# Infinidat/slimfastq

Measured on AMD Instinct MI355X. Metric: MB/s FASTQ compressed, higher is better.
Workload: dtype u8/u32 integer; 1 GPU; synthetic 10M x 150 bp Illumina reads per GPU, full qlts+gens+recs, frozen tables (one chain per lane), -l 3; level=3, block_reads=1024, prior_step=-1, blocks_per_gpu=9766, tables=frozen, chains_per_gpu=253906, raw_bytes_per_gpu=3702038404, parallelism=1 GPU

## Files before the change

slimfastq_amd/csrc/chains.hip:

```cpp
#include "kernels.h"
#include "dev_chain.h"
#include "dev_walk.h"
typedef u32 __attribute__((aligned(1))) u32_any;

#define LAST_QLT 63u
#define QROW_BYTES 256u
#define B2_INIT 0x03030303u

#define QDEC_ROW 72u
__device__ __forceinline__ void qdec_store(u16* row, u32 s, u32 cum) {
    if (s) row[8 + s - 1] = (u16)cum;
    if ((s & 7u) == 0) row[s >> 3] = (u16)cum;
    if (s == 63) row[8 + 63] = 0;
}
__global__ __launch_bounds__(256) void k_qlt_frozen_rows(const u32* __restrict__ rows66, u32 q_rows, u32* __restrict__ qrows, u16* __restrict__ qdec) {
    const u32 lane = threadIdx.x & 63;
    const u32 ctx = blockIdx.x * 4 + (threadIdx.x >> 6);
    if (ctx >= q_rows) return;
    const u32* r = rows66 + (size_t)ctx * 66;
    const u32 slot = r[lane], iend = r[65];
    if (iend == 0) {
        qrows[(size_t)ctx * 64 + lane] = (lane << 10) | (1024u << 16);
        if (qdec) qdec_store(qdec + (size_t)ctx * QDEC_ROW, lane, lane << 10);
        return;
    }
    const u32 sym = slot >> 16, fslot = lane < iend ? (slot & 0xffffu) : 0u;
    const u32 f = (u32)__builtin_amdgcn_ds_permute((int)((lane < iend ? sym : lane) * 4), (int)fslot);
    const u32 x = f + 1;
    u32 S = x;
#pragma unroll
    for (int d = 32; d > 0; d >>= 1) S += (u32)__shfl_xor((int)S, d, 64);
    u32 g = (x << 16) / S;
    g = g ? g : 1u;
    u32 sum = g, best = (g << 6) | (63u - lane);
#pragma unroll
    for (int d = 32; d > 0; d >>= 1) {
        sum += (u32)__shfl_xor((int)sum, d, 64);
        const u32 o = (u32)__shfl_xor((int)best, d, 64); best = o > best ? o : best;
    }
    if (lane == 63u - (best & 63u)) g += 65536u - sum;
    u32 incl = g;
#pragma unroll
    for (int d = 1; d < 64; d <<= 1) { const u32 o = (u32)__shfl_up((int)incl, d, 64); if (lane >= (u32)d) incl += o; }
    qrows[(size_t)ctx * 64 + lane] = (incl - g) | (g << 16);
    if (qdec) qdec_store(qdec + (size_t)ctx * QDEC_ROW, lane, incl - g);
}
void launch_qlt_frozen_rows(const u32* rows66, u32 q_rows, u32* qrows, u16* qdec, hipStream_t st) {
    hipLaunchKernelGGL(k_qlt_frozen_rows, dim3((q_rows + 3) / 4), dim3(256), 0, st, rows66, q_rows, qrows, qdec);
}

#define QH_SYMS 48u
#define QH_ROW_U16 50u
#define QH_MAP_BYTES(q_rows) ((q_rows) / 32u * 8u)
#define QH_EMPTY 0xFFFFFFFFu
__global__ __launch_bounds__(256) void k_hot_totals(const u32* __restrict__ hist, const u32* __restrict__ rows66, u32 q_rows, u32* __restrict__ ctot) {
    const u32 lane = threadIdx.x & 63;
    const u32 ctx = blockIdx.x * 4 + (threadIdx.x >> 6);
    if (ctx >= q_rows) return;
    u32 c = hist[(size_t)ctx * 64 + lane];
#pragma unroll
    for (int d = 32; d > 0; d >>= 1) c += (u32)__shfl_xor((int)c, d, 64);
    const u32 iend = rows66[(size_t)ctx * 66 + 65];
    if (lane == 0) ctot[ctx] = (iend != 0 && iend <= QH_SYMS) ? c : 0u;
}
__global__ __launch_bounds__(1024) void k_hot_select(const u32* __restrict__ ctot, u32 q_rows, u32 want, uint2* __restrict__ map, u32* __restrict__ info) {
    __shared__ u32 red[16];
    __shared__ u32 wbits[2048];
    const u32 t = threadIdx.x, lane = t & 63, wave = t >> 6;
    const u32 nwords = q_rows / 32u;
    u32 c[64];
    u32 mx = 0;
#pragma unroll
    for (u32 k = 0; k < 64; k++) {
        const u32 ctx = k * 1024u + t;
        c[k] = ctx < q_rows ? ctot[ctx] : 0u;
        mx = c[k] > mx ? c[k] : mx;
    }
    auto block_sum = [&](u32 v) {
#pragma unroll
        for (int d = 32; d > 0; d >>= 1) v += (u32)__shfl_xor((int)v, d, 64);
        __syncthreads();
        if (lane == 0) red[wave] = v;
        __syncthreads();
        u32 s2 = 0;
        for (u32 w = 0; w < 16; w++) s2 += red[w];
        return s2;
    };
    auto block_max = [&](u32 v) {
#pragma unroll
        for (int d = 32; d > 0; d >>= 1) { const u32 o = (u32)__shfl_xor((int)v, d, 64); v = o > v ? o : v; }
        __syncthreads();
        if (lane == 0) red[wave] = v;
        __syncthreads();
        u32 s2 = 0;
        for (u32 w = 0; w < 16; w++) s2 = red[w] > s2 ? red[w] : s2;
        return s2;
    };
    u32 lo = 1, hi = block_max(mx) + 1u;
    while (lo < hi) {
        const u32 mid = lo + (hi - lo) / 2u;
        u32 n = 0;
#pragma unroll
        for (u32 k = 0; k < 64; k++) n += c[k] >= mid;
        if (block_sum(n) <= want) hi = mid; else lo = mid + 1u;
    }
    const u32 T = lo;
#pragma unroll
    for (u32 k = 0; k < 64; k++) {
        const u64 m = __ballot(c[k] >= T);
        if (lane == 0) { wbits[k * 32u + wave * 2u] = (u32)m; wbits[k * 32u + wave * 2u + 1u] = (u32)(m >> 32); }
    }
    __syncthreads();
    const u32 b0 = 2u * t < nwords ? wbits[2u * t] : 0u, b1 = 2u * t + 1u < nwords ? wbits[2u * t + 1u] : 0u;
    const u32 mine = (u32)__popc(b0) + (u32)__popc(b1);
    u32 inc = mine;
#pragma unroll
    for (int d = 1; d < 64; d <<= 1) { const u32 o = (u32)__shfl_up((int)inc, d, 64); if (lane >= (u32)d) inc += o; }
    __syncthreads();
    if (lane == 63) red[wave] = inc;
    __syncthreads();
    u32 before = 0, all = 0;
    for (u32 w = 0; w < 16; w++) { const u32 v = red[w]; before += w < wave ? v : 0u; all += v; }
    const u32 rank = before + inc - mine;
    if (t == 0) info[0] = all;
    if (2u * t < nwords) map[2u * t] = make_uint2(b0, rank);
    if (2u * t + 1u < nwords) map[2u * t + 1u] = make_uint2(b1, rank + (u32)__popc(b0));
}
__global__ __launch_bounds__(256) void k_hot_image(const uint2* __restrict__ map, const u32* __restrict__ qrows, u32 q_rows, u16* __restrict__ rows) {
    const u32 lane = threadIdx.x & 63;
    const u32 ctx = blockIdx.x * 4 + (threadIdx.x >> 6);
    if (ctx >= q_rows) return;
    const uint2 mr = map[ctx >> 5];
    const u32 bit = 1u << (ctx & 31u);
    if (!(mr.x & bit)) return;
    const u32 slot = mr.y + (u32)__popc(mr.x & (bit - 1u));
    if (lane < QH_ROW_U16) rows[(size_t)slot * QH_ROW_U16 + lane] = lane <= QH_SYMS ? (u16)FZ_CUM(qrows[(size_t)ctx * 64 + lane]) : (u16)0;
}
void launch_hot_rows(const u32* hist, const u32* rows66, const u32* qrows, u32 q_rows, u32 want, u32* ctot, u8* img, u32* info, hipStream_t st) {
    hipLaunchKernelGGL(k_hot_totals, dim3((q_rows + 3) / 4), dim3(256), 0, st, hist, rows66, q_rows, ctot);
    hipLaunchKernelGGL(k_hot_select, dim3(1), dim3(1024), 0, st, (const u32*)ctot, q_rows, want, reinterpret_cast<uint2*>(img), info);
    hipLaunchKernelGGL(k_hot_image, dim3((q_rows + 3) / 4), dim3(256), 0, st, reinterpret_cast<const uint2*>(img), qrows, q_rows,
                       reinterpret_cast<u16*>(img + QH_MAP_BYTES(q_rows)));
}

#define QHD_ROW_U16 8u
#define QHD_MAX_ROWS 6000u
__global__ __launch_bounds__(256) void k_hot_totals_prior(const u32* __restrict__ rows66, u32 q_rows, u32* __restrict__ ctot) {
    const u32 ctx = blockIdx.x * 256 + threadIdx.x;
    if (ctx >= q_rows) return;
    const u32 iend = rows66[(size_t)ctx * 66 + 65];
    ctot[ctx] = iend != 0 ? rows66[(size_t)ctx * 66 + 64] + 1u : 0u;
}
__global__ __launch_bounds__(256) void k_hot_image_dec(const uint2* __restrict__ map, const u16* __restrict__ qdec, u32 q_rows, u16* __restrict__ rows) {
    const u32 ctx = blockIdx.x * 256 + threadIdx.x;
    if (ctx >= q_rows) return;
// ... 584 lines not shown
            if (w0 | w1) slice[i] = c;
            if (rows_out && last_chunk) rows_out[((size_t)b << sb) + i] = gen_row_of(c, step);
        }
        if (last_chunk) break;
        __syncthreads();
    }
    if (tid == 0) fill[b] = 0;
}
GenBins gen_bins_plan(u32 g_bits, u64 max_keys) {
    GenBins gb; gb.bins = nullptr; gb.fill = nullptr;
    gb.g_bits = g_bits;
    gb.batch = max_keys < GEN_BIN_BATCH ? (max_keys ? max_keys : 1) : GEN_BIN_BATCH;
    const u32 nb = 1u << (g_bits - gb_slice_bits(g_bits));
    gb.cap = (u32)((2ull * ((gb.batch + nb - 1) / nb) + 4096ull + 63ull) & ~63ull);
    gb.bins_bytes = (u64)gb.cap * 2ull * nb; gb.fill_bytes = 4ull * nb;
    return gb;
}
void launch_gen_count_binned(const ChainArgs& a, u32 b0, u32 b1, u64 nrec_range, u32 max_line, const GenBins& gb, u32* cnt, u32* rows_out, u32 step,
                             hipStream_t st, u32 sub) {
    const u32 g_bits = gb.g_bits, sb = gb_slice_bits(g_bits), nb = 1u << (g_bits - sb), cap = gb.cap;
    const u32 dyn2 = (2u << sb) * 4u;
    static u32 allowed = 0;
    if (dyn2 > 65536u && dyn2 > allowed) { (void)hipFuncSetAttribute(reinterpret_cast<const void*>(&k_gen_bin_count), hipFuncAttributeMaxDynamicSharedMemorySize, (int)dyn2); allowed = dyn2; }
    if (nrec_range) {
        u32 stride = gen_count_stride(nrec_range);
        if (sub == 1) { stride *= GEN_PRE; sub = 0; }
        u32 seg_len = 0;
        if (max_line >= 64u) {
            const u64 nsel = (nrec_range + stride - 1) / stride;
            for (u32 sl = 32u; sl < max_line && sl <= 512u; sl *= 2u)
                if (nsel * ((max_line + sl - 1) / sl) <= 524288ull) { seg_len = sl; break; }
        }
        if (!seg_len && max_line > 1024u) seg_len = 512u;
        const u32 segs = seg_len ? (max_line + seg_len - 1) / seg_len : 1u;
        const u64 lanes = ((nrec_range + stride - 1) / stride) * segs;
        const u64 per_lane = seg_len ? seg_len : (max_line ? max_line : 1u);
        u64 lanes_per_batch = gb.batch / per_lane; if (!lanes_per_batch) lanes_per_batch = 1;
        lanes_per_batch = (lanes_per_batch + GB_T - 1) / GB_T * GB_T;
        const u32 dyn1 = (GB_TILE + 2u * nb) * 4u;
        for (u64 id0 = 0; id0 < lanes; id0 += lanes_per_batch) {
            const u64 id1 = id0 + lanes_per_batch < lanes ? id0 + lanes_per_batch : lanes;
            const bool last = id1 >= lanes;
            hipLaunchKernelGGL(k_gen_bin, dim3((u32)((id1 - id0 + GB_T - 1) / GB_T)), dim3(GB_T), dyn1, st, a, b0, b1, stride, seg_len, segs, sub, id0, id1, g_bits, gb.bins, gb.fill, cap, cnt);
            hipLaunchKernelGGL(k_gen_bin_count, dim3(nb), dim3(1024), dyn2, st, (const u16*)gb.bins, gb.fill, cap, g_bits, cnt, last ? rows_out : nullptr, step);
        }
    } else if (rows_out) hipLaunchKernelGGL(k_gen_bin_count, dim3(nb), dim3(1024), dyn2, st, (const u16*)gb.bins, gb.fill, cap, g_bits, cnt, rows_out, step);
}

__global__ __launch_bounds__(256) void k_gen_rows(const u32* __restrict__ cnt, u32* __restrict__ rows, u64 nctx, u32 step) {
    const u64 c = (u64)blockIdx.x * 256 + threadIdx.x;
    if (c >= nctx) return;
    const uint4 n = *reinterpret_cast<const uint4*>(cnt + c * 4);
    u64 f0 = 3 + (u64)step * n.x, f1 = 3 + (u64)step * n.y, f2 = 3 + (u64)step * n.z, f3 = 3 + (u64)step * n.w;
    while ((f0 | f1 | f2 | f3) > 255) {
        f0 = (f0 >> 1) | (f0 & 1); f1 = (f1 >> 1) | (f1 & 1); f2 = (f2 >> 1) | (f2 & 1); f3 = (f3 >> 1) | (f3 & 1);
    }
    rows[c] = (u32)f0 | (u32)f1 << 8 | (u32)f2 << 16 | (u32)f3 << 24;
}
void launch_gen_rows(const u32* cnt, u32* rows, u64 nctx, u32 step, hipStream_t st) {
    hipLaunchKernelGGL(k_gen_rows, dim3((u32)((nctx + 255) / 256)), dim3(256), 0, st, cnt, rows, nctx, step);
}

__device__ __forceinline__ const u32* gen_rows_of(const ChainArgs& a, u32 b) {
    if (!a.g_ngen) return nullptr;
    u32 g = 0;
    while (g + 1 < a.g_ngen && b >= a.g_bound[g + 1]) g++;
    return a.g_rows[g];
}

#define GEN_RING 8
template <int THREADS, bool FLAT>
__global__ __launch_bounds__(THREADS) void k_gen_encode_c(ChainArgs a, u32 c0, u32 c1 ) {
    __shared__ u32 rcp[FLAT ? 1 : 1024];
    __shared__ u8 lut[256];
    __shared__ u32 ring[LaneEncB<THREADS, GEN_RING>::LDS_DWORDS];
    if constexpr (!FLAT) for (u32 i = threadIdx.x; i < 1024; i += THREADS) rcp[i] = i ? fz_recip(i) : 0u;
    for (u32 i = threadIdx.x; i < 256; i += THREADS) lut[i] = (u8)(gen_code_of(i) | (is_lower_base(i) ? 0x20u : 0u));
    __syncthreads();
    const u32 c = c0 + blockIdx.x * THREADS + threadIdx.x;
    const bool live = c < c1;
    ChainPos cp; cp.b = 0; cp.r0 = 0; cp.nrec = 0; cp.sub_lo = cp.sub_len = 0; cp.seg = 0; cp.nseg = 1;
    if (live) { cp = chain_pos(a, c); chain_seg_encode(a, cp); }
    const BlockDesc* d = &a.m.blocks[cp.b];
    LaneEncB<THREADS, GEN_RING> rc; u32 cap = 0;
    u8* outp = live ? chain_region(a, cp, SFQ_S_GEN, 3, 4, cap) : nullptr;
    rc.init(ring, threadIdx.x, outp, cap);
    const u32* rows = (!FLAT && live) ? gen_rows_of(a, cp.b) : nullptr;
    u32 illegal = 0;
    if (a.flat_quads && (FLAT || !__any(rows != nullptr))) {
        illegal = walk_bases_q(a, cp.r0, cp.nrec, live ? d->solid : 0u, lut,
            [&](u32 sym, u32 k) { const u32 bits = 2u * k; rc.encode_bits_if(k ? ~0u : 0u, sym & ((1u << bits) - 1u), 1u, bits); rc.drain(); },
            a.exc_flag, cp.sub_lo, cp.sub_len);
    } else if (FLAT || !__any(rows != nullptr)) {
        const u32 r12 = fz_recip(12u);
        illegal = walk_bases_b(a, cp.r0, cp.nrec, live ? d->solid : 0u, 0u, lut, [&](u32, u32) {},
            [&](u32, u32 code, u32 vm) { rc.encode_if(vm, 3u * code, 3u, 12u, r12); },
            [&]() { rc.drain(); }, a.exc_flag, cp.sub_lo, cp.sub_len);
    } else if constexpr (!FLAT) {
        const u32* rp = rows ? rows : a.g_init;
        const u32 mask = (live && rows) ? (1u << d->gen_bits) - 1u : 0u;
        u32 rv[16];
        illegal = walk_bases_b(a, cp.r0, cp.nrec, live ? d->solid : 0u, mask, lut,
            [&](u32 j, u32 ctx) { rv[j] = rp[ctx]; },
            [&](u32 j, u32 code, u32 vm) {
                const u32 v = rv[j];
                const u32 f0 = v & 0xff, f1 = (v >> 8) & 0xff, f2 = (v >> 16) & 0xff, f3 = v >> 24;
                const u32 tot = (f0 + f1) + (f2 + f3);
                const u32 below = v & ((1u << (8 * code)) - 1u);
                const u32 cum = (below & 0xff) + ((below >> 8) & 0xff) + (below >> 16);
                rc.encode_if(vm, cum, (v >> (8 * code)) & 0xff, tot, rcp[tot]);
            },
            [&]() { rc.drain(); }, a.exc_flag, cp.sub_lo, cp.sub_len);
    }
    if (live) {
        a.csz[c] = rc.finish();
        if (rc.err & 2) atomicMax(&a.m.blocks[cp.b].status, (u32)(-SFQ_E_OVERFLOW));
        else if (rc.err) atomicMax(&a.m.blocks[cp.b].status, (u32)(-SFQ_E_CORRUPT));
        if (illegal) atomicMax(&a.m.blocks[cp.b].status, (u32)(-SFQ_E_GENCHAR));
    }
}
__device__ __forceinline__ uint4 gp_below(u32 n) {
    const u64 lo = n >= 8u ? ~0ull : (1ull << (8u * n)) - 1ull;
    const u64 hi = n >= 16u ? ~0ull : n <= 8u ? 0ull : (1ull << (8u * (n - 8u))) - 1ull;
    return make_uint4((u32)lo, (u32)(lo >> 32), (u32)hi, (u32)(hi >> 32));
}
__device__ __forceinline__ uint4 gp_load16(const u8* buf, u64 nbytes, long long at) {
    if (at >= 0 && (u64)at + 16u <= nbytes) return load16(buf, nbytes, (u64)at);
    u32 w[4] = {0, 0, 0, 0};
    for (u32 i = 0; i < 16; i++) { const long long p = at + (long long)i; if (p >= 0 && (u64)p < nbytes) w[i >> 2] |= (u32)buf[p] << ((i & 3) * 8); }
    return make_uint4(w[0], w[1], w[2], w[3]);
}
__device__ __forceinline__ u32 gp_codes(u32 w, u32 valid, u32& odd, u32& ill) {
    const u32 s1 = w >> 1;
    u32 cd = (s1 ^ (w >> 2)) & 0x03030303u;
    const u32 want = __builtin_amdgcn_perm(0u, 0x47544341u, s1 & 0x03030303u);
    odd = 0; ill = 0;
    if ((want ^ w) & valid) {
        cd = 0;
#pragma unroll
        for (u32 i = 0; i < 4; i++) {
            const u32 ch = (w >> (8u * i)) & 0xffu, g = gen_code_of(ch);
            cd |= (g & 3u) << (8u * i);
            if ((valid >> (8u * i)) & 0xffu) {
                if (g > 3u || is_lower_base(ch)) odd |= 0x80u << (8u * i);
                if (g & 0x10u) ill = 1;
            }
        }
    }
    return cd & valid & 0x03030303u;
}
__device__ __forceinline__ u32 gp_fold(u32 cd) { return cd | (cd >> 6); }
__device__ __forceinline__ u32 gp_nib(u32 t) { return ((t >> 7) * 0x01020408u) >> 24; }
__device__ __forceinline__ u32 gp_bits16(u32 o0, u32 o1, u32 o2, u32 o3) { return gp_nib(o0) | gp_nib(o1) << 4 | gp_nib(o2) << 8 | gp_nib(o3) << 12; }
__global__ __launch_bounds__(256) void k_gen_pack_raw(ChainArgs a, u32 c0, u32 c1) {
    const u32 lane = threadIdx.x & 63u;
    const u32 c = c0 + blockIdx.x * 4u + (threadIdx.x >> 6);
    if (c >= c1) return;
    ChainPos cp = chain_pos(a, c); chain_seg_encode(a, cp);
    const u32 solid = a.m.blocks[cp.b].solid;
    u32 cap = 0;
    u32* out = reinterpret_cast<u32*>(chain_region(a, cp, SFQ_S_GEN, 3, 4, cap));
    const u8* buf = a.st_off ? a.st_buf : a.m.fq;
    const u64 nbytes = a.st_off ? a.st_bytes : a.nbytes;
    u32 done = 0;
    u32 carry = 0;
    u32 illegal = 0;
    for (u32 k0 = 0; k0 < cp.nrec; k0 += 64u) {
        const u32 k = k0 + lane;
        u64 b0 = 0, b1 = 0;
        if (k < cp.nrec) {
            const u64 r = cp.r0 + k;
            if (a.st_off) { b0 = a.st_off[r]; b1 = b0 + a.st_len[r]; }
            else { b0 = a.m.line_off[4 * r + 1] + solid; b1 = a.m.line_off[4 * r + 2] - 1; }
            if (cp.sub_len) {
                if (b1 < b0) b1 = b0;
                const u64 lo = b0 + cp.sub_lo;
                b0 = lo < b1 ? lo : b1;
                b1 = b0 + cp.sub_len < b1 ? b0 + cp.sub_len : b1;
            }
            if (b1 < b0) b1 = b0;
        }
        const u32 len = (u32)(b1 - b0);
        u32 inc = len;
#pragma unroll
        for (int d = 1; d < 64; d <<= 1) { const u32 o = (u32)__shfl_up((int)inc, d, 64); if (lane >= (u32)d) inc += o; }
        const u32 st = inc - len;
        const u32 tot = (u32)__shfl((int)inc, 63, 64);
        const u32 end = done + tot;
        const bool last_chunk = k0 + 64u >= cp.nrec;
        const u32 t0 = done >> 4, t1 = (end + 15u) >> 4;
        for (u32 tb = t0; tb < t1; tb += 64u) {
            const u32 t = tb + lane;
            const u32 d0 = 16u * t;
            const u32 lo = d0 > done ? d0 : done, hi = d0 + 16u < end ? d0 + 16u : end;
            u32 kr = 0;
#pragma unroll
            for (u32 s = 32; s > 0; s >>= 1) { const u32 sk = (u32)__shfl((int)st, (int)(kr + s), 64); if (sk + done <= lo) kr += s; }
            uint4 w = make_uint4(0, 0, 0, 0);
            u32 pos = lo;
            while (__any(pos < hi)) {
                const u32 ks = kr & 63u;
                const u32 sk = (u32)__shfl((int)st, (int)ks, 64) + done, lk = (u32)__shfl((int)len, (int)ks, 64);
                const u64 bk = (u64)__shfl((unsigned long long)b0, (int)ks, 64);
                const u32 e = sk + lk < hi ? sk + lk : hi;
                if (pos < hi && e > pos) {
                    const u32 j = pos - d0;
                    const uint4 v = gp_load16(buf, nbytes, (long long)(bk + (pos - sk)) - (long long)j);
                    const uint4 m0 = gp_below(j), m1 = gp_below(j + (e - pos));
                    w.x = (w.x & ~(m1.x & ~m0.x)) | (v.x & m1.x & ~m0.x);
                    w.y = (w.y & ~(m1.y & ~m0.y)) | (v.y & m1.y & ~m0.y);
                    w.z = (w.z & ~(m1.z & ~m0.z)) | (v.z & m1.z & ~m0.z);
                    w.w = (w.w & ~(m1.w & ~m0.w)) | (v.w & m1.w & ~m0.w);
                    pos = e;
                }
                kr++;
            }
            const bool any = lo < hi;
            const uint4 va = gp_below(any ? hi - d0 : 0u), vb = gp_below(any ? lo - d0 : 0u);
            const uint4 vm = make_uint4(va.x & ~vb.x, va.y & ~vb.y, va.z & ~vb.z, va.w & ~vb.w);
            u32 o0, o1, o2, o3, i0, i1, i2, i3;
            const u32 f0 = gp_fold(gp_codes(w.x, vm.x, o0, i0)), f1 = gp_fold(gp_codes(w.y, vm.y, o1, i1));
            const u32 f2 = gp_fold(gp_codes(w.z, vm.z, o2, i2)), f3 = gp_fold(gp_codes(w.w, vm.w, o3, i3));
            illegal |= i0 | i1 | i2 | i3;
            u32 p01 = __builtin_amdgcn_perm(f1, f0, 0x06020400u), p23 = __builtin_amdgcn_perm(f3, f2, 0x06020400u);
            p01 |= p01 >> 12; p23 |= p23 >> 12;
            u32 code = __builtin_amdgcn_perm(p23, p01, 0x05040100u);
            if (t == t0) code |= carry;
            u32 odd = gp_bits16(o0, o1, o2, o3);
            if (a.exc_flag) {
                while (__any(odd != 0u)) {
                    const u32 jb = odd ? (u32)__builtin_ctz(odd) : 0u;
                    u32 ko = 0;
#pragma unroll
                    for (u32 s = 32; s > 0; s >>= 1) { const u32 sk = (u32)__shfl((int)st, (int)(ko + s), 64); if (sk + done <= d0 + jb) ko += s; }
                    const u32 ke = (u32)__shfl((int)inc, (int)ko, 64) + done;
                    if (odd) {
                        a.exc_flag[cp.r0 + k0 + ko] = 1;
                        odd &= ke - d0 >= 16u ? 0u : ~((1u << (ke - d0)) - 1u);
                    }
                }
            }
            const bool held = t == t1 - 1u && (end & 15u) && !last_chunk;
            if (t < t1 && !held && 4u * t < cap) out[t] = code;
            if (!last_chunk) carry = (end & 15u) ? (u32)__shfl((int)code, (int)((t1 - 1u - tb) & 63u), 64) : 0u;
        }
        done = end;
    }
    if (lane == 0) {
        const u32 n = (done + 3u) >> 2;
        a.csz[c] = n;
        if (n > cap) atomicMax(&a.m.blocks[cp.b].status, (u32)(-SFQ_E_OVERFLOW));
    }
    if (__any(illegal != 0u) && lane == 0) atomicMax(&a.m.blocks[cp.b].status, (u32)(-SFQ_E_GENCHAR));
}
void launch_gen_encode_c(const ChainArgs& a, hipStream_t st, u32 c0, u32 c1, bool flat) {
    constexpr int T = 256;
    if (!c1 || c1 > a.geo.nchains) c1 = a.geo.nchains;
    if (c1 <= c0) return;
    if (a.flat_raw) { hipLaunchKernelGGL(k_gen_pack_raw, dim3((c1 - c0 + 3) / 4), dim3(256), 0, st, a, c0, c1); return; }
    const dim3 grid((c1 - c0 + T - 1) / T);
    if (flat) hipLaunchKernelGGL((k_gen_encode_c<T, true>), grid, dim3(T), 0, st, a, c0, c1);
    else hipLaunchKernelGGL((k_gen_encode_c<T, false>), grid, dim3(T), 0, st, a, c0, c1);
}

__device__ __forceinline__ u32 b2_pick(u32 v, LaneDecQ& rc, const u32* rcp) {
    const u32 f0 = v & 0xff, f1 = (v >> 8) & 0xff, f2 = (v >> 16) & 0xff, f3 = v >> 24;
    const u32 c1 = f0, c2 = f0 + f1, c3 = c2 + f2, tot = c3 + f3;
    u32 r;
    const u32 prob = rc.get_freq(tot, rcp[tot], r);
    const u32 b = (prob >= c1 ? 1u : 0u) + (prob >= c2 ? 1u : 0u) + (prob >= c3 ? 1u : 0u);
    const u32 cum = b == 0 ? 0u : b == 1 ? c1 : b == 2 ? c2 : c3;
    rc.decode(r, cum, (v >> (8 * b)) & 0xff);
    return b;
}
template <int THREADS>
__global__ __launch_bounds__(THREADS) void k_gen_decode_c(ChainArgs a, DecodeArgs da, u32 c0, u32 c1 ) {
    __shared__ u32 rcp[1024];
    for (u32 i = threadIdx.x; i < 1024; i += THREADS) rcp[i] = i ? fz_recip(i) : 0u;
    __syncthreads();
    const u32 c = c0 + blockIdx.x * THREADS + threadIdx.x;
    if (c >= c1) return;
    ChainPos cp = chain_pos(a, c);
    const BlockDesc* d = &a.m.blocks[cp.b];
    LaneDecQ rc; rc.init(da.streams + a.coff[c], a.csz[c], reinterpret_cast<const u8*>(a.qesc));
    const u32* rows = gen_rows_of(a, cp.b);
    const u32 alphabet = d->solid ? 0x33323130u  : 0x54474341u ;
    const u32 mask = (1u << d->gen_bits) - 1u;
    const u32 INIT = 0x007616c7u;
    const u32 r12 = fz_recip(12u);
    u32 n_next = cp.nrec ? da.slen[cp.r0] : 0u; u64 off_next = cp.nrec ? da.soff[cp.r0] : 0ull;
    if (a.seg_len) {
        const u32 ql = da.qlen[cp.r0];
        seg_range(cp, ql > n_next ? ql : n_next);
        const u64 lo = cp.sub_lo < n_next ? cp.sub_lo : n_next;
        n_next = (u32)(n_next - lo < cp.sub_len ? n_next - lo : cp.sub_len); off_next += lo;
    }
    const u8* const raw = da.streams + a.coff[c]; const u32 raw_n = a.csz[c];
    u32 racc = 0, rnb = 0, rat = 0, rbad = 0;
    for (u32 k = 0; k < cp.nrec; k++) {
        const u32 llen = n_next; const u64 off = off_next;
        if (k + 1 < cp.nrec) { n_next = da.slen[cp.r0 + k + 1]; off_next = da.soff[cp.r0 + k + 1]; }
        LaneOut32 out; out.begin(da.seq_stage + off);
        u32 last = INIT;
        if (a.flat_raw) {
            for (u32 i = 0; i < llen; i++) {
                if (rnb == 0) {
                    if (rat + 4u <= raw_n) { racc = *reinterpret_cast<const u32_any*>(raw + rat); rat += 4u; rnb = 32u; }
                    else if (rat < raw_n) { racc = raw[rat++]; rnb = 8u; }
                    else { rbad = 1; racc = 0; rnb = 32u; }
                }
                out.put((alphabet >> (8u * (racc & 3u))) & 0xffu);
                racc >>= 2; rnb -= 2u;
            }
        } else
        if (rows) {
            u32 v = rows[last & mask];
            for (u32 i = 0; i < llen; i++) {
                const uint4 cand = *reinterpret_cast<const uint4*>(rows + ((last << 2) & mask));
                rc.top_up();
                const u32 b = b2_pick(v, rc, rcp);
                out.put((alphabet >> (8 * b)) & 0xff);
                last = (last << 2) | b;
                v = b == 0 ? cand.x : b == 1 ? cand.y : b == 2 ? cand.z : cand.w;
            }
        } else if (a.flat_quads) {
            for (u32 i = 0; i < llen; i += 4u) {
                const u32 k = llen - i < 4u ? llen - i : 4u;
                rc.top_up();
                u32 r;
                const u32 S = rc.get_freq_bits(2u * k, r);
                rc.decode1(r, S, 1u);
                for (u32 j = 0; j < k; j++) out.put((alphabet >> (8u * ((S >> (2u * j)) & 3u))) & 0xffu);
            }
        } else {
            for (u32 i = 0; i < llen; i++) {
                rc.top_up();
                u32 r;
                const u32 prob = rc.get_freq(12u, r12, r);
                const u32 b = (prob >= 3u ? 1u : 0u) + (prob >= 6u ? 1u : 0u) + (prob >= 9u ? 1u : 0u);
                rc.decode1(r, 3u * b, 3u);
                out.put((alphabet >> (8 * b)) & 0xff);
            }
        }
        out.end();
    }
    if (a.flat_raw) { if (rbad || rat != raw_n || (rnb >= 8u) || racc) atomicMax(&a.m.blocks[cp.b].status, (u32)(-SFQ_E_CORRUPT)); }
    else
    if (rc.err) atomicMax(&a.m.blocks[cp.b].status, (u32)(-SFQ_E_CORRUPT));
}
void launch_gen_decode_c(const ChainArgs& a, const DecodeArgs& da, u32 c0, u32 c1, hipStream_t st) {
    constexpr int T = 256;
    if (c1 > a.geo.nchains) c1 = a.geo.nchains;
    if (c1 <= c0) return;
    hipLaunchKernelGGL(k_gen_decode_c<T>, dim3((c1 - c0 + T - 1) / T), dim3(T), 0, st, a, da, c0, c1);
}

#include "dev_rec_lane.h"
#include "dev_wave.h"

struct RecChainPos { u32 b; u64 r0; u32 nrec; };
__device__ __forceinline__ RecChainPos rec_chain_pos(const ChainArgs& a, u32 c) {
    RecChainPos p;
    p.b = c / a.rgeo.cpb;
    const u32 j = c - p.b * a.rgeo.cpb;
    const BlockDesc* d = &a.m.blocks[p.b];
    const u32 k0 = j * a.rgeo.chain_reads;
    p.nrec = k0 < d->nrec ? (d->nrec - k0 < a.rgeo.chain_reads ? d->nrec - k0 : a.rgeo.chain_reads) : 0u;
    p.r0 = d->rec0 + k0;
    return p;
}
__device__ __forceinline__ u8* rec_chain_region(const ChainArgs& a, const RecChainPos& p, u32& cap) {
    const BlockDesc* d = &a.m.blocks[p.b];
    const u64 t0 = a.m.line_off[4 * d->rec0], tc = a.m.line_off[4 * p.r0], te = a.m.line_off[4 * (p.r0 + p.nrec)];
    const u64 lo = ((tc - t0) * 3 / 2 + 3) & ~3ull, hi = ((te - t0) * 3 / 2) & ~3ull;
    cap = hi > lo ? (u32)(hi - lo) : 0u;
    return a.m.arena + d->out_off[SFQ_S_REC] + lo;
}

#define REC_HBUF 128u
#define REC_LDS_ROWS 8u
struct RecFrozenEnc {
    static constexpr bool inband = true;
    const u32* rows; LaneEnc rc;
    u8* lbuf;
    const u16* lmap; const u32* lrows;
    __device__ __forceinline__ void record(u32) {}
    __device__ __forceinline__ const u8* stage(const u8* g, u32 n, u32 k) {
        if (n + 1 > REC_HBUF) return g;
        u8* dst = lbuf + (k & 1u) * REC_HBUF;
        const u32 nw = (n + 4) / 4;
#pragma unroll 8
        for (u32 i = 0; i < nw; i++) reinterpret_cast<u32*>(dst)[i] = reinterpret_cast<const u32_any*>(g)[i];
        return dst;
    }
    __device__ __forceinline__ void put(u32 row, u32 sym) {
        const u32 slot = lmap[row];
        const u32 e = slot != 0xFFFFu ? lrows[slot * 256 + sym] : rows[(size_t)row * 256 + sym];
// ... 1141 lines not shown
```

Before: 331,100 MB/s.

## Add uniform-length fast path to raw gen packing kernel

When every read in a 64-record chunk has the same length, the gen pack kernel skips the wave prefix scan and binary-search shuffles. It locates records with reciprocal division and reads record offsets from shared memory. Each 16-byte output dword spans at most two records and is assembled with byte perms. A branchless ACGT code path is used, with a shared LUT fallback only for unusual characters. Loads skip bounds checks when the whole chunk is safely in range, and some shuffles become readlane. This adds code complexity and a second path that must match the general one bit for bit.

Result: faster. 357,400 MB/s, median of 6 (+7.9%).

```diff
diff --git a/slimfastq_amd/csrc/chains.hip b/slimfastq_amd/csrc/chains.hip
--- a/slimfastq_amd/csrc/chains.hip
+++ b/slimfastq_amd/csrc/chains.hip
@@ -1,6 +1,7 @@
 #include "kernels.h"
 #include "dev_chain.h"
 #include "dev_walk.h"
+#include "gp_uniform.h"
 typedef u32 __attribute__((aligned(1))) u32_any;
 
 #define LAST_QLT 63u
@@ -891,9 +892,68 @@
 __device__ __forceinline__ u32 gp_fold(u32 cd) { return cd | (cd >> 6); }
 __device__ __forceinline__ u32 gp_nib(u32 t) { return ((t >> 7) * 0x01020408u) >> 24; }
 __device__ __forceinline__ u32 gp_bits16(u32 o0, u32 o1, u32 o2, u32 o3) { return gp_nib(o0) | gp_nib(o1) << 4 | gp_nib(o2) << 8 | gp_nib(o3) << 12; }
+__device__ __forceinline__ u32 gp_codes4(u32 w, u32& x) {
+    const u32 sm = (w >> 1) & 0x03030303u;
+    x = __builtin_amdgcn_perm(0u, 0x47544341u, sm) ^ w;
+    return __builtin_amdgcn_perm(0u, 0x02030100u, sm);
+}
+__device__ __forceinline__ u32 gp_lut_of(u32 c) {
+    const u32 g = gen_code_of(c);
+    return (g & 3u) | ((g > 3u || is_lower_base(c)) ? 0x80u : 0u) | ((g & 0x10u) ? 0x40u : 0u);
+}
+__device__ __forceinline__ u32 gp_lut4(const u8* lut, u32 w) {
+    return (u32)lut[w & 0xffu] | (u32)lut[(w >> 8) & 0xffu] << 8 | (u32)lut[(w >> 16) & 0xffu] << 16 | (u32)lut[w >> 24] << 24;
+}
+#define GP_PACK_MUL ((1u << 24) | (1u << 18) | (1u << 12) | (1u << 6))
+struct GpUni { const u8* buf; u64 nbytes; const u64* tb0; const u8* lut; u32 L, rcp, done, end; bool safe; };
+template <bool FULL>
+__device__ __forceinline__ u32 gp_uniform_dword(const GpUni& u, u32 d0, u32& odd, u32& ill) {
+    u32 lo = d0, hi = d0 + 16u;
+    if constexpr (!FULL) { lo = d0 > u.done ? d0 : u.done; hi = d0 + 16u < u.end ? d0 + 16u : u.end; }
+    uint4 w = make_uint4(0x41414141u, 0x41414141u, 0x41414141u, 0x41414141u);
+    if (FULL || lo < hi) {
+        const u32 j = lo - d0;
+        const GpPiece p = gp_uniform_piece(lo - u.done, hi - u.done, j, u.L, u.rcp);
+        const long long at = (long long)(u.tb0[p.kr] + p.off) - (long long)j;
+        if (u.safe) { const u32* q = reinterpret_cast<const u32*>(u.buf + at); w = make_uint4(q[0], q[1], q[2], q[3]); }
+        else w = gp_load16(u.buf, u.nbytes, at);
+        if (p.two) {
+            const long long at2 = (long long)u.tb0[p.kr + 1u] - (long long)p.cut;
+            uint4 v;
+            if (u.safe) { const u32* q = reinterpret_cast<const u32*>(u.buf + at2); v = make_uint4(q[0], q[1], q[2], q[3]); }
+            else v = gp_load16(u.buf, u.nbytes, at2);
+            const u32 c4 = p.cut * 0x01010101u;
+            const u32 s0 = (((0x83828180u - c4) >> 5) & 0x04040404u) | 0x03020100u, s1 = (((0x87868584u - c4) >> 5) & 0x04040404u) | 0x03020100u;
+            const u32 s2 = (((0x8b8a8988u - c4) >> 5) & 0x04040404u) | 0x03020100u, s3 = (((0x8f8e8d8cu - c4) >> 5) & 0x04040404u) | 0x03020100u;
+            w.x = __builtin_amdgcn_perm(v.x, w.x, s0); w.y = __builtin_amdgcn_perm(v.y, w.y, s1);
+            w.z = __builtin_amdgcn_perm(v.z, w.z, s2); w.w = __builtin_amdgcn_perm(v.w, w.w, s3);
+        }
+        if constexpr (!FULL) {
+            const uint4 va = gp_below(hi - d0), vb = gp_below(j);
+            const uint4 vm = make_uint4(va.x & ~vb.x, va.y & ~vb.y, va.z & ~vb.z, va.w & ~vb.w);
+            w.x = (w.x & vm.x) | (0x41414141u & ~vm.x); w.y = (w.y & vm.y) | (0x41414141u & ~vm.y);
+            w.z = (w.z & vm.z) | (0x41414141u & ~vm.z); w.w = (w.w & vm.w) | (0x41414141u & ~vm.w);
+        }
+    }
+    u32 x0, x1, x2, x3;
+    u32 cd0 = gp_codes4(w.x, x0), cd1 = gp_codes4(w.y, x1), cd2 = gp_codes4(w.z, x2), cd3 = gp_codes4(w.w, x3);
+    odd = 0; ill = 0;
+    if (__any((x0 | x1 | x2 | x3) != 0u)) {
+        if (__any(x0 != 0u)) { if (x0) { const u32 e = gp_lut4(u.lut, w.x); cd0 = e & 0x03030303u; odd |= gp_nib(e & 0x80808080u); ill |= e & 0x40404040u; } }
+        if (__any(x1 != 0u)) { if (x1) { const u32 e = gp_lut4(u.lut, w.y); cd1 = e & 0x03030303u; odd |= gp_nib(e & 0x80808080u) << 4; ill |= e & 0x40404040u; } }
+        if (__any(x2 != 0u)) { if (x2) { const u32 e = gp_lut4(u.lut, w.z); cd2 = e & 0x03030303u; odd |= gp_nib(e & 0x80808080u) << 8; ill |= e & 0x40404040u; } }
+        if (__any(x3 != 0u)) { if (x3) { const u32 e = gp_lut4(u.lut, w.w); cd3 = e & 0x03030303u; odd |= gp_nib(e & 0x80808080u) << 12; ill |= e & 0x40404040u; } }
+    }
+    return __builtin_amdgcn_perm(cd1 * GP_PACK_MUL, cd0 * GP_PACK_MUL, 0x0c0c0703u) | __builtin_amdgcn_perm(cd3 * GP_PACK_MUL, cd2 * GP_PACK_MUL, 0x07030c0cu);
+}
 __global__ __launch_bounds__(256) void k_gen_pack_raw(ChainArgs a, u32 c0, u32 c1) {
+    __shared__ u8 lut[256];
+    __shared__ u64 tb0s[4][64];
+    lut[threadIdx.x] = (u8)gp_lut_of(threadIdx.x);
+    __syncthreads();
     const u32 lane = threadIdx.x & 63u;
-    const u32 c = c0 + blockIdx.x * 4u + (threadIdx.x >> 6);
+    u64* tb0 = tb0s[threadIdx.x >> 6];
+    const u32 c = (u32)__builtin_amdgcn_readfirstlane((int)(c0 + blockIdx.x * 4u + (threadIdx.x >> 6)));
     if (c >= c1) return;
     ChainPos cp = chain_pos(a, c); chain_seg_encode(a, cp);
     const u32 solid = a.m.blocks[cp.b].solid;
@@ -920,13 +980,55 @@
             if (b1 < b0) b1 = b0;
         }
         const u32 len = (u32)(b1 - b0);
+        const bool last_chunk = k0 + 64u >= cp.nrec;
+        const u32 L = (u32)__builtin_amdgcn_readfirstlane((int)len);
+        if (L >= GP_UNI_MIN_LEN && L <= GP_UNI_MAX_LEN && __all(k >= cp.nrec || len == L)) {
+            const u32 nk = cp.nrec - k0 < 64u ? cp.nrec - k0 : 64u;
+            const u32 end = done + L * nk;
+            tb0[lane] = b0;
+            __builtin_amdgcn_fence(__ATOMIC_RELEASE, "wavefront");
+            __builtin_amdgcn_wave_barrier();
+            __builtin_amdgcn_fence(__ATOMIC_ACQUIRE, "wavefront");
+            GpUni u;
+            u.buf = buf; u.nbytes = nbytes; u.tb0 = tb0; u.lut = lut; u.L = L; u.rcp = gp_uniform_recip(L); u.done = done; u.end = end;
+            u.safe = __all(k >= cp.nrec || (b0 >= 16u && b1 + 16u <= nbytes));
+            const u32 cin = carry;
+            carry = 0;
+            const u32 t0 = done >> 4, t1 = (end + 15u) >> 4;
+            for (u32 tb = t0; tb < t1; tb += 64u) {
+                const u32 t = tb + lane;
+                const u32 d0 = 16u * t;
+                const bool full = 16u * tb >= done && 16u * (tb + 64u) <= end;
+                u32 odd, ill, code;
+                if (full) code = gp_uniform_dword<true>(u, d0, odd, ill);
+                else { code = gp_uniform_dword<false>(u, d0, odd, ill); if (t == t0) code |= cin; }
+                illegal |= ill;
+                if (a.exc_flag && __any(odd != 0u)) {
+                    while (odd) {
+                        u32 off;
+                        const u32 ko = gp_uniform_rec(d0 + (u32)__builtin_ctz(odd) - done, L, u.rcp, off);
+                        a.exc_flag[cp.r0 + k0 + ko] = 1;
+                        const u32 ke = done + (ko + 1u) * L;
+                        odd &= ke - d0 >= 16u ? 0u : ~((1u << (ke - d0)) - 1u);
+                    }
+                }
+                if (full) { if (4u * t < cap) out[t] = code; }
+                else {
+                    const bool held = t == t1 - 1u && (end & 15u) && !last_chunk;
+                    if (t < t1 && !held && 4u * t < cap) out[t] = code;
+                    if (!last_chunk && (end & 15u) && tb + 64u >= t1) carry = (u32)__builtin_amdgcn_readlane((int)code, (int)((t1 - 1u - tb) & 63u));
+                }
+            }
+            __builtin_amdgcn_wave_barrier();
+            done = end;
+            continue;
+        }
         u32 inc = len;
 #pragma unroll
         for (int d = 1; d < 64; d <<= 1) { const u32 o = (u32)__shfl_up((int)inc, d, 64); if (lane >= (u32)d) inc += o; }
         const u32 st = inc - len;
-        const u32 tot = (u32)__shfl((int)inc, 63, 64);
+        const u32 tot = (u32)__builtin_amdgcn_readlane((int)inc, 63);
         const u32 end = done + tot;
-        const bool last_chunk = k0 + 64u >= cp.nrec;
         const u32 t0 = done >> 4, t1 = (end + 15u) >> 4;
         for (u32 tb = t0; tb < t1; tb += 64u) {
             const u32 t = tb + lane;
@@ -981,7 +1083,7 @@
             }
             const bool held = t == t1 - 1u && (end & 15u) && !last_chunk;
             if (t < t1 && !held && 4u * t < cap) out[t] = code;
-            if (!last_chunk) carry = (end & 15u) ? (u32)__shfl((int)code, (int)((t1 - 1u - tb) & 63u), 64) : 0u;
+            if (!last_chunk) carry = (end & 15u) ? (u32)__builtin_amdgcn_readlane((int)code, (int)((t1 - 1u - tb) & 63u)) : 0u;
         }
         done = end;
     }
diff --git a/slimfastq_amd/csrc/gp_uniform.h b/slimfastq_amd/csrc/gp_uniform.h
--- /dev/null
+++ b/slimfastq_amd/csrc/gp_uniform.h
@@ -0,0 +1,29 @@
+#pragma once
+#include <stdint.h>
+#if defined(__HIPCC__) || defined(__CUDACC__)
+#define GP_HD __host__ __device__ __forceinline__
+#else
+#define GP_HD inline
+#endif
+
+#define GP_UNI_MIN_LEN 16u
+#define GP_UNI_MAX_LEN (1u << 24)
+
+GP_HD uint32_t gp_uniform_recip(uint32_t L) { return 0xffffffffu / L; }
+
+GP_HD uint32_t gp_uniform_rec(uint32_t rel, uint32_t L, uint32_t rcp, uint32_t& off) {
+    uint32_t kr = (uint32_t)(((uint64_t)rel * rcp) >> 32);
+    off = rel - kr * L;
+    if (off >= L) { kr++; off -= L; }
+    return kr;
+}
+
+struct GpPiece { uint32_t kr, off, cut; bool two; };
+GP_HD GpPiece gp_uniform_piece(uint32_t lo, uint32_t hi, uint32_t j, uint32_t L, uint32_t rcp) {
+    GpPiece p;
+    p.kr = gp_uniform_rec(lo, L, rcp, p.off);
+    const uint32_t n1 = L - p.off;
+    p.two = n1 < hi - lo;
+    p.cut = j + (p.two ? n1 : hi - lo);
+    return p;
+}
```
